# Luke-TS/3360-ray-tracer

Measured on AMD Instinct MI355X. Metric: Mrays/s (primary+secondary) at fixed spp; RMS pixel error vs CPU ref, higher is better.
Workload: dtype f64; 1 GPU; c3_bunny: bunny scene 1000x562, 200 spp, depth 20, fixed spp; scene_prims=69452, bvh_nodes=40541, mode=persistent, precision=fast, schedule=park, framebuffer=pinned host, frame_rows_covered=True, parallelism=tile-split x1 (interleaved 4-row stripes, no collectives)

## Files before the change

### 3360-ray-tracer_amd/csrc/rtx_device.h

```cpp
#pragma once

#include <hip/hip_runtime.h>
#include <stdint.h>

#include <type_traits>

#include "rtx.h"

#ifndef RTX_PARK_TU
#define RTX_PARK_TU 0
#endif

namespace rtxd {

constexpr bool kSincosSmall = !RTX_PARK_TU;
constexpr bool kTriBranchless = RTX_PARK_TU;
constexpr bool kEarlyTex = !RTX_PARK_TU;
constexpr bool kLeafStep = RTX_PARK_TU;

constexpr double kPi = 3.14159265358979323846;
constexpr double kInf = __builtin_inf();

struct V3 {
  double x, y, z;
// ... 333 lines not shown
  mat_out = R.mat;
  const PrimRec* P = &R;
  const int kind = KIND >= 0 ? KIND : P->kind;
  if (kTriBranchless && KIND >= 0 && kind == RTX_PRIM_TRIANGLE) {
    const V3 A{P->g[0], P->g[1], P->g[2]};
    const V3 e1 = tri_e1(P->g), e2 = tri_e2(P->g);
    const V3 pvec = cross(d, e2);
    const float det = (float)dot(e1, pvec);
    const float inv_det = 1.0f / det;
    const V3 tvec = o - A;
    const float u = (float)(dot(tvec, pvec) * (double)inv_det);
    const V3 qvec = cross(tvec, e1);
    const float v = (float)(dot(d, qvec) * (double)inv_det);
    const float t = (float)(dot(e2, qvec) * (double)inv_det);
    const bool ok = !(fabsf(det) < 1e-6f) & !(u < 0.0f || u > 1.0f) & !(v < 0.0f || (u + v) > 1.0f) &
                    !((double)t < tmin || (double)t > tmax);
    t_out = (double)t;
    return ok;
  }
  if (kind == RTX_PRIM_TRIANGLE) {
    V3 A{P->g[0], P->g[1], P->g[2]};
    V3 e1 = tri_e1(P->g), e2 = tri_e2(P->g);
    V3 pvec = cross(d, e2);
    float det = (float)dot(e1, pvec);
    if (fabsf(det) < 1e-6f) return false;
    float inv_det = 1.0f / det;
    V3 tvec = o - A;
    float u = (float)(dot(tvec, pvec) * (double)inv_det);
    if (u < 0.0f || u > 1.0f) return false;
    V3 qvec = cross(tvec, e1);
    float v = (float)(dot(d, qvec) * (double)inv_det);
    if (v < 0.0f || (u + v) > 1.0f) return false;
    float t = (float)(dot(e2, qvec) * (double)inv_det);
    if ((double)t < tmin || (double)t > tmax) return false;
    t_out = (double)t;
    return true;
  }
  if (kind == RTX_PRIM_SPHERE) {
    V3 c{P->g[0], P->g[1], P->g[2]};
    double radius = fmax(0.0, P->g[3]);
    V3 oc = c - o;
    double a = len2(d);
    double h = dot(d, oc);
    double cc = len2(oc) - radius * radius;
    double disc = h * h - a * cc;
    if (disc < 0) return false;
    double sq = sqrt(disc);
    double root = (h - sq) / a;
    if (!(tmin < root && root < tmax)) {
      root = (h + sq) / a;
      if (!(tmin < root && root < tmax)) return false;
    }
    t_out = root;
    return true;
  }
  int ax, a0, a1;
  if (kind == RTX_PRIM_XY_RECT) ax = 2, a0 = 0, a1 = 1;
  else if (kind == RTX_PRIM_XZ_RECT) ax = 1, a0 = 0, a1 = 2;
  else ax = 0, a0 = 1, a1 = 2;
  double t = (P->g[4] - comp(o, ax)) / comp(d, ax);
  if (!(tmin < t && t < tmax)) return false;
  double x = comp(o, a0) + t * comp(d, a0);
  double y = comp(o, a1) + t * comp(d, a1);
  if (x < P->g[0] || x > P->g[1] || y < P->g[2] || y > P->g[3]) return false;
  t_out = t;
  return true;
}

__device__ __forceinline__ bool prim_t(const rtx_prim* __restrict__ P, bool tris, V3 o, V3 d, double tmin,
                                       double tmax, double& t_out) {
  int32_t m;
  return prim_t(P, tris, o, d, tmin, tmax, t_out, m);
}

template <bool UV = true>
__device__ __forceinline__ void finish_hit(const DScene& S, int64_t best, V3 o, V3 d, double tmin, Hit& h) {
  h.u = 0.0, h.v = 0.0;
  hit_prim<UV>(S.prims + best, o, d, tmin, kInf, h);
  h.lazy_uv = (!UV && S.prims[best].kind == RTX_PRIM_SPHERE) ? best : -1;
}

template <bool UV = true>
__device__ __forceinline__ void finish_hit_at(const DScene& S, int64_t best, double t, V3 o, V3 d, Hit& h) {
  const rtx_prim* __restrict__ P = S.prims + best;
  const int kind = P->kind;
  h.u = 0.0, h.v = 0.0;
  h.mat = P->material;
  h.t = t;
  h.lazy_uv = -1;
  if (kind == RTX_PRIM_SPHERE) {
    const V3 c{P->g[0], P->g[1], P->g[2]};
    const double radius = fmax(0.0, P->g[3]);
    h.p = o + h.t * d;
    const V3 outward = (h.p - c) / radius;
    set_face_normal(h, d, outward);
    if (UV) sphere_uv(outward, h.u, h.v);
    else h.lazy_uv = best;
  } else if (kind == RTX_PRIM_TRIANGLE) {
    h.p = o + h.t * d;
    if (S.tri_n) {
      const double2 n01 = *(const double2*)(S.tri_n + 4 * best), n2 = *(const double2*)(S.tri_n + 4 * best + 2);
      set_face_normal(h, d, V3{n01.x, n01.y, n2.x});
    } else {
      const V3 e1 = tri_e1(P->g), e2 = tri_e2(P->g);
      set_face_normal(h, d, normalize(cross(e1, e2)));
    }
  } else {
    int a0, a1;
    V3 n;
    if (kind == RTX_PRIM_XY_RECT) a0 = 0, a1 = 1, n = v3(0, 0, 1);
    else if (kind == RTX_PRIM_XZ_RECT) a0 = 0, a1 = 2, n = v3(0, 1, 0);
    else a0 = 1, a1 = 2, n = v3(1, 0, 0);
    if (UV) {
      const double x = comp(o, a0) + t * comp(d, a0);
      const double y = comp(o, a1) + t * comp(d, a1);
      h.u = (x - P->g[0]) / (P->g[1] - P->g[0]);
      h.v = (y - P->g[2]) / (P->g[3] - P->g[2]);
    } else {
      h.lazy_uv = best;
    }
    set_face_normal(h, d, n);
    h.p = o + h.t * d;
  }
}

__device__ __forceinline__ bool box_hit(const double* lo, const double* hi, V3 o, V3 inv_unused, V3 d,
                                        double tmin, double tmax) {
#pragma unroll
  for (int a = 0; a < 3; a++) {
    const double adinv = 1.0 / comp(d, a);
    double t0 = (lo[a] - comp(o, a)) * adinv;
    double t1 = (hi[a] - comp(o, a)) * adinv;
    if (t0 < t1) {
      if (t0 > tmin) tmin = t0;
      if (t1 < tmax) tmax = t1;
    } else {
      if (t1 > tmin) tmin = t1;
      if (t0 < tmax) tmax = t0;
    }
    if (tmax <= tmin) return false;
  }
  return true;
}

struct Counters {
  uint32_t nodes, prims;
  uint32_t wnodes, wprims;
  uint32_t tris, sphs;
  uint32_t witers, widle;
  uint32_t wlive;
};
struct CountersClk : Counters {
  uint64_t t_top, t_seg, t_walk, t_leaf;
  uint64_t cyc_refill, cyc_walk, cyc_shade, cyc_leaf;
  uint32_t wshade, lshade;
};
__device__ __forceinline__ void count_prim(Counters& c, const rtx_prim* P) {
  c.prims++;
  const int k = P->kind;
  c.tris += k == RTX_PRIM_TRIANGLE ? 1u : 0u;
  c.sphs += k == RTX_PRIM_SPHERE ? 1u : 0u;
}
__device__ __forceinline__ bool first_active_lane() {
  const unsigned long long m = __ballot(1);
  return (int)__lane_id() == __ffsll((long long)m) - 1;
}

template <int STACK, bool COUNT>
__device__ __forceinline__ int64_t trace_parity(const DScene& S, V3 o, V3 d, double tmin, double tmax,
                                                uint32_t* stk, int stride, Counters& cnt, double& t_best) {
  int64_t best = -1;
  double closest = tmax, t;
  if (!S.use_bvh) {
    for (int64_t i = 0; i < S.n_prims; i++) {
      if (COUNT) count_prim(cnt, S.prims + i);
      if (prim_t(S.prims + i, S.has_tris, o, d, tmin, closest, t)) closest = t, best = i;
    }
    t_best = closest;
    return best;
  }
  int sp = 0;
  stk[0] = 0u;
  sp = 1;
  while (sp > 0) {
    const uint32_t ni = stk[(--sp) * stride];
    const rtx_bvh_node* __restrict__ nd = S.nodes + ni;
    double lo[3] = {nd->lo[0], nd->lo[1], nd->lo[2]};
    double hi[3] = {nd->hi[0], nd->hi[1], nd->hi[2]};
    const uint32_t a = nd->left_first, b = nd->right_count, leaf = nd->is_leaf;
    if (COUNT) cnt.nodes++;
    if (!box_hit(lo, hi, o, o, d, tmin, closest)) continue;
    if (leaf) {
      for (uint32_t i = 0; i < b; i++) {
        if (COUNT) count_prim(cnt, S.prims + a + i);
        if (prim_t(S.prims + a + i, S.has_tris, o, d, tmin, closest, t)) closest = t, best = (int64_t)a + i;
      }
    } else {
      if (sp + 2 > STACK) __builtin_trap();
      stk[(sp++) * stride] = b;
      stk[(sp++) * stride] = a;
    }
  }
  t_best = closest;
  return best;
}

__device__ __forceinline__ float f32_round_up(double x) {
  float f = (float)x;
  if ((double)f < x) f = __int_as_float(__float_as_int(f) + (f >= 0.0f ? 1 : -1));
  return f;
}

__device__ __forceinline__ void pin(double& x) { asm volatile("" : "+v"(x)); }
__device__ __forceinline__ void pin(V3& v) {
  pin(v.x);
  pin(v.y);
  pin(v.z);
}

__device__ __forceinline__ void fray4_axis_signed(double o, double d, int axis, float& inv, float& nl, float& nh,
                                                  uint32_t& off) {
  inv = __builtin_amdgcn_rcpf((float)d);
  const float n0 = -((float)o * inv);
  off = 32u * axis;
  if (!(fabsf(n0) < __builtin_inff())) {
    inv = 0.0f, nl = -__builtin_inff(), nh = __builtin_inff();
    return;
  }
  const float delta = fabsf(n0) * 0x1p-20f;
  nl = n0 - delta, nh = n0 + delta;
  if (inv < 0.0f) off += 16u;
}
__device__ __forceinline__ float f4c(const float4& v, int c) { return c == 0 ? v.x : (c == 1 ? v.y : (c == 2 ? v.z : v.w)); }

__device__ __forceinline__ void cswap4(float& ta, int32_t& ca, float& tb, int32_t& cb) {
  const bool s = tb < ta;
  const float t = s ? tb : ta;
  tb = s ? ta : tb;
  ta = t;
  const int32_t c = s ? cb : ca;
  cb = s ? ca : cb;
  ca = c;
}

struct FRay4L {
  float iex, iey, iez, nex, ney, nez;
  float ixx, ixy, ixz, nxx, nxy, nxz;
  uint32_t ox, oy, oz;
};
struct FRay4 {
  float ix, iy, iz, nlx, nhx, nly, nhy, nlz, nhz;
  uint32_t ox, oy, oz;
};
__device__ __forceinline__ FRay4L make_fray4l(V3 o, V3 d) {
  FRay4 b;
  fray4_axis_signed(o.x, d.x, 0, b.ix, b.nlx, b.nhx, b.ox);
  fray4_axis_signed(o.y, d.y, 1, b.iy, b.nly, b.nhy, b.oy);
  fray4_axis_signed(o.z, d.z, 2, b.iz, b.nlz, b.nhz, b.oz);
  constexpr float lo = 0.99999f, hi = 1.00001f;
  FRay4L r;
  r.iex = b.ix * lo, r.iey = b.iy * lo, r.iez = b.iz * lo;
  r.nex = b.nlx * lo, r.ney = b.nly * lo, r.nez = b.nlz * lo;
  r.ixx = b.ix * hi, r.ixy = b.iy * hi, r.ixz = b.iz * hi;
  r.nxx = b.nhx * hi, r.nxy = b.nhy * hi, r.nxz = b.nhz * hi;
  r.ox = b.ox, r.oy = b.oy, r.oz = b.oz;
  return r;
}

struct TravState {
  uint32_t node;
  int32_t sp;
  double closest;
  int32_t best;
  int32_t mat;
  float tmax_f;
};
__device__ __forceinline__ void trav_init(TravState& ts, double tmax) {
  ts.node = 0, ts.sp = 0, ts.closest = tmax, ts.best = -1, ts.mat = -1;
  ts.tmax_f = f32_round_up(tmax);
}

constexpr int32_t kGlobalSpheres = 4;
__device__ __forceinline__ bool sphere_root(double a, double h, double sq, double tmin, double tmax, double& root) {
  const double n1 = h - sq;
  const bool near_first = !(a > 0.0 && a < kInf && tmin >= 0.0) || n1 > 0.0;
  root = (near_first ? n1 : h + sq) / a;
  bool ok = tmin < root && root < tmax;
  if (!ok && near_first) {
    root = (h + sq) / a;
    ok = tmin < root && root < tmax;
  }
  return ok;
}
template <bool COUNT, bool SPHERES = true>
__device__ __forceinline__ void trav_globals(const DScene& S, V3 o, V3 d, double tmin, Counters& cnt, TravState& ts) {
  if (SPHERES && (S.n_global & kGlobalSpheres)) {
    typedef uint32_t u4 __attribute__((ext_vector_type(4)));
    typedef double d2 __attribute__((ext_vector_type(2)));
    typedef const __attribute__((address_space(4))) u4 cu4;
    typedef const __attribute__((address_space(4))) d2 cd2;
    for (int i = 0; i < (S.n_global & 3); i++) {
      const uintptr_t P = (uintptr_t)(S.prims + (uint32_t)S.global[i]);
      const u4 w0 = *(cu4*)P;
      const d2 w1 = *((cd2*)P + 1), w2 = *((cd2*)P + 2);
      if (COUNT) {
        cnt.prims++, cnt.sphs++;
// ... 291 lines not shown
}

__device__ __forceinline__ V3 tex_value(const DScene& S, int32_t t, const Hit& rec) {
  double u = rec.u, v = rec.v;
  const V3 p = rec.p;
  for (int guard = 0; guard < 16; guard++) {
    const rtx_texture T = S.texs[t];
    if (T.kind == RTX_TEX_SOLID) return v3(T.color[0], T.color[1], T.color[2]);
    if (T.kind == RTX_TEX_CHECKER) {
      int xi = (int)floor(T.inv_scale * p.x);
      int yi = (int)floor(T.inv_scale * p.y);
      int zi = (int)floor(T.inv_scale * p.z);
      t = ((xi + yi + zi) % 2 == 0) ? T.even : T.odd;
      continue;
    }
    if (T.image < 0) return v3(0, 1, 1);
    const DImage im = S.images[T.image];
    if (im.h <= 0) return v3(0, 1, 1);
    if (rec.lazy_uv >= 0) {
      const double2 uv = lazy_uv(S.prims + rec.lazy_uv, p);
      u = uv.x, v = uv.y;
    }
    u = u < 0 ? 0 : (u > 1 ? 1 : u);
    v = 1.0 - (v < 0 ? 0 : (v > 1 ? 1 : v));
    int i = (int)(u * im.w);
    int j = (int)(v * im.h);
    i = i < 0 ? 0 : (i < im.w ? i : im.w - 1);
    j = j < 0 ? 0 : (j < im.h ? j : im.h - 1);
    const uint8_t* px = im.texels + ((size_t)j * im.w + i) * 3;
    double s = 1.0 / 255.0;
    return v3(s * px[0], s * px[1], s * px[2]);
  }
  return v3(0, 1, 1);
}

__device__ __forceinline__ V3 mat_tex(const DScene& S, const rtx_material& m, const Hit& rec) {
  if (m.texture < 0) return v3(m.albedo[0], m.albedo[1], m.albedo[2]);
  return tex_value(S, m.texture, rec);
}

__device__ __forceinline__ double pow5(double x) {
  const double p2 = x * x, e2 = fma(x, x, -p2);
  const double p4 = p2 * p2, e4 = fma(p2, p2, -p4) + 2.0 * (p2 * e2);
  const double p5 = p4 * x, e5 = fma(p4, x, -p5) + e4 * x;
  return p5 + e5;
}

__device__ __forceinline__ double reflectance(double c, double ri) {
  double r0 = (1.0 - ri) / (1.0 + ri);
  r0 = r0 * r0;
  return r0 + (1.0 - r0) * pow5(1.0 - c);
}

__device__ __forceinline__ bool mat_scatter(const DScene& S, const rtx_material& m, V3 rin_d, const Hit& rec,
                                            V3& att, V3& sd, Rng& g) {
  if (m.kind == RTX_MAT_LAMBERTIAN) {
    V3 dir = rec.normal + random_unit_vector(g);
    if (near_zero(dir)) dir = rec.normal;
    sd = dir;
    att = mat_tex(S, m, rec);
    return true;
  }
  if (m.kind == RTX_MAT_METAL) {
    V3 r = reflect(rin_d, rec.normal);
    r = r + m.fuzz * random_unit_vector(g);
    sd = r;
    att = v3(m.albedo[0], m.albedo[1], m.albedo[2]);
    return dot(sd, rec.normal) > 0;
  }
  if (m.kind == RTX_MAT_DIELECTRIC) {
    att = v3(1.0, 1.0, 1.0);
    double eta = rec.front_face ? (1.0 / m.ref_idx) : m.ref_idx;
    V3 ud = normalize(rin_d);
    double ct = fmin(dot(-ud, rec.normal), 1.0);
    double stt = sqrt(1.0 - ct * ct);
    bool cannot = eta * stt > 1.0;
    if (cannot || reflectance(ct, eta) > g.next()) sd = reflect(ud, rec.normal);
    else sd = refract(ud, rec.normal, eta);
    return true;
  }
  return false;
}

__device__ __forceinline__ V3 mat_emitted(const DScene& S, const rtx_material& m, const Hit& rec) {
  if (m.kind == RTX_MAT_DIFFUSE_LIGHT) return mat_tex(S, m, rec);
  return v3(0, 0, 0);
}
template <bool NOTEX>
__device__ __forceinline__ V3 mat_tex_t(const DScene& S, const rtx_material& m, const Hit& rec) {
  if (NOTEX) return v3(m.albedo[0], m.albedo[1], m.albedo[2]);
  return mat_tex(S, m, rec);
}
template <bool NOTEX>
__device__ __forceinline__ V3 mat_emitted_t(const DScene& S, const rtx_material& m, const Hit& rec) {
  if (m.kind == RTX_MAT_DIFFUSE_LIGHT) return mat_tex_t<NOTEX>(S, m, rec);
  return v3(0, 0, 0);
}

__device__ __forceinline__ V3 sky(V3 d) {
  V3 ud = normalize(d);
  double t = 0.5 * (ud.y + 1.0);
  return (1.0 - t) * v3(1.0, 1.0, 1.0) + t * v3(0.5, 0.7, 1.0);
}

template <bool NODOF = false>
__device__ __forceinline__ void get_ray(const rtx_camera& c, int i, int j, Rng& g, V3& o, V3& d) {
  double oy = g.next() - 0.5;
  double ox = g.next() - 0.5;
  V3 p00{c.pixel00[0], c.pixel00[1], c.pixel00[2]};
  V3 du{c.pixel_delta_u[0], c.pixel_delta_u[1], c.pixel_delta_u[2]};
  V3 dv{c.pixel_delta_v[0], c.pixel_delta_v[1], c.pixel_delta_v[2]};
  V3 ps = p00 + ((i + ox) * du) + ((j + oy) * dv);
  V3 center{c.center[0], c.center[1], c.center[2]};
  if (NODOF || c.defocus_angle <= 0) {
    o = center;
  } else {
    V3 p = random_in_unit_disk(g);
    V3 ddu{c.defocus_disk_u[0], c.defocus_disk_u[1], c.defocus_disk_u[2]};
    V3 ddv{c.defocus_disk_v[0], c.defocus_disk_v[1], c.defocus_disk_v[2]};
    o = center + (p.x * ddu) + (p.y * ddv);
  }
  d = ps - o;
}

struct Path {
  V3 o, d, thr;
  int32_t depth;
};

__device__ __forceinline__ V3 normalize_l(V3 v, double& l) {
  l = sqrt(len2(v));
  if (l == 0.0) return {0, 0, 0};
  return v / l;
}

enum : int32_t {
  kShadeEmit = 0,
  kShadeDead = 1,
  kShadeDiffuse = 2,
  kShadeSpecular = 3
};
struct ShadeOut {
  V3 f;
  float ct, pdf;
  int32_t what;
  int32_t fsrc;
};
template <class T>
__device__ __forceinline__ const T* opaque(const T* p) {
  asm volatile("" : "+v"(p));
  return p;
}

template <bool LAMB = false, bool NOTEX = false, bool SET_ORIGIN = true, bool DEFER_F = false>
__device__ __forceinline__ void shade_core(const DScene& S, int max_depth, Path& p, const Hit& rec, bool hit, Rng& g,
                                           const rtx_material& m, ShadeOut& so) {
  static_assert(!DEFER_F || NOTEX, "deferred BSDF values need texture-free shading");
  so.what = kShadeDead;
  so.fsrc = 0;
  double lnd;
  const V3 nd = normalize_l(p.d, lnd);
  if (!hit || p.depth >= max_depth) {
    const double t = 0.5 * (nd.y + 1.0);
    so.f = (1.0 - t) * v3(1.0, 1.0, 1.0) + t * v3(0.5, 0.7, 1.0);
    so.what = kShadeEmit;
    return;
  }
  if (!LAMB) {
    V3 em = mat_emitted_t<NOTEX>(S, m, rec);
    if (!near_zero(em)) {
      so.f = em;
      so.what = kShadeEmit;
      return;
    }
  }
  const int kind = LAMB ? (int)RTX_MAT_LAMBERTIAN : m.kind;
  const bool isL = kind == RTX_MAT_LAMBERTIAN, isM = kind == RTX_MAT_METAL, isG = kind == RTX_MAT_DIELECTRIC;
  if (!(isL || isM || isG)) return;
  const V3 n = rec.normal;
  V3 ftex = v3(0, 0, 0);
  if (kEarlyTex && !NOTEX && !DEFER_F && isL) ftex = mat_tex_t<NOTEX>(S, m, rec);
  double r1 = 0.0, r2 = 0.0;
  if (isL) r1 = g.next(), r2 = g.next();
  V3 ru = v3(0, 0, 0);
  if (isM) ru = random_unit_vector(g);
  double l1;
  V3 s1 = normalize_l(isL ? n : nd, l1);
  pin(s1);
  const V3 w = s1;
  const V3 win = (!isL && l1 == 0.0) ? v3(-0.0, -0.0, -0.0) : s1;
  double eta = 0.0, ci = 0.0, a2 = 0.0;
  if (isG) {
    eta = rec.front_face ? m.albedo[0] : m.ref_idx;
    ci = dot(win, n);
    ci = ci < -1.0 ? -1.0 : (ci > 1.0 ? 1.0 : ci);
    a2 = fmax(0.0, 1.0 - ci * ci);
  }
  double s2 = sqrt(isL ? r2 : a2);
  pin(s2);
  double x = 0.0, y = 0.0;
  if (isL) {
    const double phi = 2.0 * kPi * r1;
    double cph, sph;
    cos_sin<kSincosSmall || !LAMB>(phi, cph, sph);
    x = s2 * cph;
    y = s2 * sph;
  }
  bool g_reflect = false;
  V3 perp = v3(0, 0, 0);
  double a3 = 1.0;
  if (isG) {
    const double st = eta * s2;
    g_reflect = st >= 1.0;
    if (!g_reflect) {
      const double r0 = m.albedo[1];
      const double Fr = r0 + (1.0 - r0) * pow5(1.0 - fabs(ci));
      g_reflect = g.next() < Fr;
    }
    if (!g_reflect) {
      const double c = fmin(dot(-win, n), 1.0);
      perp = eta * (win + c * n);
      a3 = fabs(1.0 - len2(perp));
    }
  }
  double s3 = sqrt(isL ? 1.0 - r2 : a3);
  pin(s3);
  V3 in4;
  if (isL) {
    const V3 a = (fabs(w.x) > 0.9) ? v3(0, 1, 0) : v3(1, 0, 0);
    in4 = cross(w, a);
  } else {
    in4 = reflect(nd, n);
    in4 = in4 + m.fuzz * ru;
  }
  double l4;
  V3 s4 = normalize_l(in4, l4);
  pin(s4);
  V3 wi;
  if (isL) {
    const V3 v = s4;
    const V3 u = cross(v, w);
    wi = normalize(x * u + y * v + s3 * w);
    if (dot(wi, n) <= 0) return;
    const float cf = (float)dot(n, wi);
    const float pdf = (cf <= 0.0f) ? 0.0f : (float)((double)cf / kPi);
    if (DEFER_F) so.fsrc = 1;
    else so.f = ((kEarlyTex && !NOTEX) ? ftex : mat_tex_t<NOTEX>(S, m, rec)) / kPi;
    if (pdf < 1e-6f) return;
    so.ct = fmaxf(0.0f, (float)dot(wi, n));
    so.pdf = pdf;
    so.what = kShadeDiffuse;
  } else if (isM) {
    wi = s4;
    if (dot(wi, n) <= 0) return;
    if (DEFER_F) so.fsrc = 2;
    else so.f = v3(m.albedo[0], m.albedo[1], m.albedo[2]);
    so.what = kShadeSpecular;
  } else {
    if (g_reflect) {
      wi = reflect(win, n);
      so.f = v3(1.0, 1.0, 1.0);
    } else {
      const V3 par = (-s3) * n;
      wi = perp + par;
      const double k = eta * eta;
      so.f = v3(k, k, k);
    }
    so.what = kShadeSpecular;
  }
  if (SET_ORIGIN) p.o = rec.p;
  p.d = wi, p.depth = p.depth + 1;
}

__device__ __forceinline__ bool shade_finish(const ShadeOut& so, V3& thr, int32_t depth, Rng& g, V3& L,
                                             const rtx_material* m = nullptr) {
  L = v3(0, 0, 0);
  if (so.what == kShadeEmit) {
    L = L + thr * so.f;
    return false;
  }
  if (so.what == kShadeDead) return false;
  V3 f = so.f;
  if (so.fsrc) {
    const rtx_material* mp = opaque(m);
    f = v3(mp->albedo[0], mp->albedo[1], mp->albedo[2]);
    if (so.fsrc == 1) f = f / kPi;
  }
  V3 c = so.what == kShadeDiffuse ? ((double)so.ct * (thr * f)) / (double)so.pdf : thr * f;
  if (depth > 5) {
    double q = fmax(fmax(c.x, c.y), c.z);
    q = q < 0.1 ? 0.1 : (q > 0.95 ? 0.95 : q);
    if (g.next() > q) return false;
    c = c / q;
  }
  thr = c;
  return true;
}

template <bool LAMB = false, bool NOTEX = false>
__device__ __forceinline__ bool shade_merged(const DScene& S, int max_depth, Path& p, const Hit& rec, bool hit,
                                             Rng& g, V3& L, const rtx_material& m) {
  ShadeOut so;
  shade_core<LAMB, NOTEX>(S, max_depth, p, rec, hit, g, m, so);
  return shade_finish(so, p.thr, p.depth, g, L);
}

template <bool LAMB = false, bool NOTEX = false>
__device__ __forceinline__ bool shade(const DScene& S, int max_depth, Path& p, const Hit& rec, bool hit, Rng& g,
                                      V3& L, const rtx_material& m) {
  return shade_merged<LAMB, NOTEX>(S, max_depth, p, rec, hit, g, L, m);
}

__device__ __forceinline__ bool shade(const DScene& S, int max_depth, Path& p, const Hit& rec, bool hit, Rng& g,
                                      V3& L) {
  rtx_material m;
  if (hit) m = S.mats[rec.mat];
  return shade(S, max_depth, p, rec, hit, g, L, m);
}

}
```

### 3360-ray-tracer_amd/csrc/rtx_kernels.h

```cpp
#pragma once

#include "rtx_device.h"

namespace rtxd {

constexpr int kBlock = 256;

constexpr int kTraceWaves = 4;
constexpr int kSlotTargetLog2 = 29;
constexpr int kRefillMin = 24;
constexpr int kRefillMinPark = 12;
constexpr int kParkAt = 16;
constexpr int kChunkPlain = 256, kChunkPark = 512;
constexpr int kChunkSharedPlain = 256, kChunkSharedPark = 128;
static_assert(kChunkSharedPlain <= 511 && kChunkSharedPark <= 511, "ChunkLds keeps a chunk's size in 9 bits");

struct FastDiv {
  uint32_t m, sh;
  __host__ __device__ __forceinline__ uint32_t div(uint32_t n) const {
    const uint32_t t = (uint32_t)(((uint64_t)n * m) >> 32);
    return (t + ((n - t) >> (sh & 0xFFu))) >> (sh >> 8);
  }
};
inline FastDiv make_fastdiv(uint32_t d) {
  if (d <= 1) return FastDiv{0u, 0u};
  uint32_t l = 0;
  while (l < 32 && (1ull << l) < d) l++;
  const uint64_t m = ((((uint64_t)1 << 32) * (((uint64_t)1 << l) - d)) / d) + 1;
  return FastDiv{(uint32_t)m, 1u | ((l - 1) << 8)};
}

struct PixelMap {
  int32_t W, H;
  int32_t stripes;
  int32_t x0, y0, w, h;
  int32_t srows, sidx, scount;
  FastDiv frow, fsrows;
  template <bool FD = true>
  __host__ __device__ __forceinline__ void xy(uint32_t local, int& x, int& y) const {
    if (!stripes) {
      const uint32_t r = FD ? frow.div(local) : local / (uint32_t)w;
      x = x0 + (int)(local - r * (uint32_t)w);
      y = y0 + (int)r;
    } else {
      const uint32_t r = FD ? frow.div(local) : local / (uint32_t)W;
      x = (int)(local - r * (uint32_t)W);
      const uint32_t blk = FD ? fsrows.div(r) : r / (uint32_t)srows;
      y = ((int)blk * scount + sidx) * srows + (int)(r - blk * (uint32_t)srows);
    }
  }
};
inline void set_map_div(PixelMap& m) {
  const int row = m.stripes ? m.W : m.w;
  m.frow = make_fastdiv((uint32_t)(row > 1 ? row : 1));
  m.fsrows = make_fastdiv((uint32_t)(m.srows > 1 ? m.srows : 1));
}

struct PathQueue {
  double *ox, *oy, *oz, *dx, *dy, *dz, *tx, *ty, *tz;
  uint32_t* slot;
  uint32_t* meta;
  int32_t* hit;
};

struct RenderArgs {
  DScene S;
  rtx_camera cam;
  PixelMap map;
  uint64_t seed;
  int64_t npix;
  int32_t K;
  FastDiv fK;
  int32_t s0;
  int32_t max_depth;
  int32_t scatter_api;
  const uint8_t* conv;
  double* L;
  unsigned long long* counters;
  int32_t stack_slots;
};

__device__ __forceinline__ void store_radiance(const RenderArgs& A, uint32_t slot, V3 L) {
  double* Lp = A.L + 3 * (uint64_t)slot;
  __builtin_nontemporal_store(L.x, Lp), __builtin_nontemporal_store(L.y, Lp + 1), __builtin_nontemporal_store(L.z, Lp + 2);
}

__device__ __forceinline__ uint32_t lane_id() { return __lane_id(); }

__device__ __forceinline__ int64_t wave_compact(bool want, unsigned int* counter) {
  const unsigned long long mask = __ballot(want);
  if (mask == 0) return -1;
  const int leader = __ffsll((long long)mask) - 1;
  const int total = __popcll(mask);
  unsigned int base = 0;
  if ((int)lane_id() == leader) base = atomicAdd(counter, (unsigned int)total);
  base = __shfl(base, leader);
  const int rank = __popcll(mask & ((1ull << lane_id()) - 1ull));
  return want ? (int64_t)base + rank : -1;
}

constexpr size_t stack_lds_bytes(int STACK) { return (size_t)(STACK + 1) * kBlock * sizeof(uint32_t); }
struct PersistLds {
  uint32_t stack, thr, hitp, leafq, block, end;
};

struct PixelSoA {
  double *sum, *mean, *m2;
  int32_t* samples;
  uint8_t* conv;
};

constexpr bool spec_walk(int park, bool fast, bool scatter) { return park == 2 && fast && !scatter; }
constexpr int64_t kSpecMaxNodes = 65536;
struct ChunkLds {
  unsigned long long w[kBlock / 64];
};
constexpr uint32_t block_region_bytes(int kind) { return kind == 1 ? (uint32_t)sizeof(ChunkLds) : 0u; }
constexpr int block_region_kind(int map, bool scatter) { return map == 1 && !scatter ? 1 : 0; }
constexpr PersistLds persist_lds(int stack_slots, bool spec, int block_region = 0) {
  const uint32_t stack_bytes = (uint32_t)stack_slots * kBlock * (spec ? 2u : 4u);
  const uint32_t thr = (stack_bytes + 7u) & ~7u, hitp = thr + 3u * kBlock * 8u, leafq = hitp + 3u * kBlock * 8u;
  const uint32_t tl = leafq + (spec ? (uint32_t)kLeafQueue * kBlock * 4u : 0u);
  return PersistLds{0u, thr, hitp, leafq, tl, tl + block_region_bytes(block_region)};
}

template <int STACK, bool FAST, bool COUNT, int TK = -1>
__device__ __forceinline__ int64_t trace(const DScene& S, V3 o, V3 d, double tmin, double tmax, uint32_t* stk,
                                         Counters& c, double& t_best, int32_t& mat_best) {
  if (FAST) return trace_fast4_lean<STACK, COUNT, TK>(S, o, d, tmin, tmax, stk, kBlock, c, t_best, mat_best);
  const int64_t b = trace_parity<STACK, COUNT>(S, o, d, tmin, tmax, stk, kBlock, c, t_best);
  mat_best = b >= 0 ? S.prims[b].material : -1;
  return b;
}
template <int STACK, bool FAST, bool COUNT>
__device__ __forceinline__ int64_t trace(const DScene& S, V3 o, V3 d, double tmin, double tmax, uint32_t* stk,
                                         Counters& c, double& t_best) {
  int32_t m;
  return trace<STACK, FAST, COUNT>(S, o, d, tmin, tmax, stk, c, t_best, m);
}

__device__ __forceinline__ void flush_clock(const RenderArgs& A, const CountersClk& c) {
  if (c.cyc_refill) atomicAdd(&A.counters[18], c.cyc_refill);
  if (c.cyc_walk) atomicAdd(&A.counters[19], c.cyc_walk);
  if (c.cyc_shade) atomicAdd(&A.counters[20], c.cyc_shade);
  if (c.wshade) atomicAdd(&A.counters[21], (unsigned long long)c.wshade);
  if (c.lshade) atomicAdd(&A.counters[22], (unsigned long long)c.lshade);
  if (c.cyc_leaf) atomicAdd(&A.counters[23], c.cyc_leaf);
}
__device__ __forceinline__ void flush_counters(const RenderArgs& A, const Counters& c, uint32_t segs,
                                               uint32_t prims, bool count) {
  if (count) {
    atomicAdd(&A.counters[2], (unsigned long long)c.nodes);
    atomicAdd(&A.counters[3], (unsigned long long)c.prims);
    atomicAdd(&A.counters[4], (unsigned long long)c.wnodes);
    atomicAdd(&A.counters[5], (unsigned long long)c.wprims);
    atomicAdd(&A.counters[6], (unsigned long long)c.tris);
    atomicAdd(&A.counters[7], (unsigned long long)c.sphs);
    if (c.witers) atomicAdd(&A.counters[10], (unsigned long long)c.witers);
    if (c.widle) atomicAdd(&A.counters[11], (unsigned long long)c.widle);
    if (c.wlive) atomicAdd(&A.counters[12], (unsigned long long)c.wlive);
  }
  if (segs) atomicAdd(&A.counters[0], (unsigned long long)segs);
  if (prims) atomicAdd(&A.counters[1], (unsigned long long)prims);
}

template <int STACK, bool FAST>
__global__ __launch_bounds__(kBlock, kTraceWaves) void k_intersect(DScene S, const rtx_ray* __restrict__ rays,
                                                                       int64_t n, rtx_hit* __restrict__ hits,
                                                                       double tmin, double tmax) {
  extern __shared__ __attribute__((aligned(16))) uint32_t lds[];
  uint32_t* stk = lds + threadIdx.x;
  const int64_t i = (int64_t)blockIdx.x * kBlock + threadIdx.x;
  if (i >= n) return;
  const rtx_ray r = rays[i];
  V3 o{r.origin[0], r.origin[1], r.origin[2]}, d{r.direction[0], r.direction[1], r.direction[2]};
  Counters c{};
  double tb;
  const int64_t best = trace<STACK, FAST, false>(S, o, d, tmin, tmax, stk, c, tb);
  rtx_hit out;
  out.pad_ = 0;
  if (best >= 0) {
    Hit h;
    finish_hit_at(S, best, tb, o, d, h);
    out.hit = 1;
    out.front_face = h.front_face, out.material = h.mat, out.t = h.t;
    out.p[0] = h.p.x, out.p[1] = h.p.y, out.p[2] = h.p.z;
    out.normal[0] = h.normal.x, out.normal[1] = h.normal.y, out.normal[2] = h.normal.z;
    out.u = h.u, out.v = h.v;
  } else {
    out.hit = 0, out.front_face = 0, out.material = -1, out.t = 0;
    out.p[0] = out.p[1] = out.p[2] = 0;
    out.normal[0] = out.normal[1] = out.normal[2] = 0;
    out.u = out.v = 0;
  }
  hits[i] = out;
}


template <int STACK, bool FAST, bool COUNT>
__global__ __launch_bounds__(kBlock, kTraceWaves) void k_wf_extend(RenderArgs A, PathQueue q,
                                                                       const unsigned int* count) {
  extern __shared__ __attribute__((aligned(16))) uint32_t lds[];
  uint32_t* stk = lds + threadIdx.x;
  const int64_t n = *count;
  Counters c{};
  uint32_t segs = 0;
  for (int64_t i = (int64_t)blockIdx.x * kBlock + threadIdx.x; i < n; i += (int64_t)gridDim.x * kBlock) {
    const V3 o = v3(q.ox[i], q.oy[i], q.oz[i]);
    const V3 d = v3(q.dx[i], q.dy[i], q.dz[i]);
    double tb;
    q.hit[i] = (int32_t)trace<STACK, FAST, COUNT>(A.S, o, d, (double)0.001f, kInf, stk, c, tb);
    segs++;
  }
  flush_counters(A, c, segs, 0, COUNT);
}



template <int STACK, bool FAST, bool COUNT, bool SCATTER, int PARK, int TK = -1, bool LAMB = false,
          bool NOTEX = false, bool NODOF = false, int MAP = 0>
__global__ __launch_bounds__(kBlock, kTraceWaves) void k_persistent(RenderArgs A, unsigned long long* next_slot) {
  extern __shared__ __attribute__((aligned(16))) uint32_t lds[];
  constexpr bool kSpecLds = spec_walk(PARK, FAST, SCATTER);
  constexpr bool kShared = block_region_kind(MAP, SCATTER) == 1;
  static_assert((PARK > 0) == (RTX_PARK_TU != 0), "k_persistent: PARK kernels belong to rtx_park.hip");
  constexpr int kChunk = PARK ? kChunkPark : kChunkPlain;
  constexpr int kChunkShared = PARK ? kChunkSharedPark : kChunkSharedPlain;
  const PersistLds lay = persist_lds(A.stack_slots, kSpecLds, block_region_kind(MAP, SCATTER));
  char* const ldsb = (char*)lds;
  if (COUNT && threadIdx.x == 0) atomicMax(&A.counters[13], ~(unsigned long long)wall_clock64());
  unsigned long long* const cw = (unsigned long long*)(ldsb + lay.block);
  (void)cw;
  if (kShared) {
    if (threadIdx.x < kBlock / 64) cw[threadIdx.x] = 0ull;
    __syncthreads();
  }
  uint32_t* stk = (uint32_t*)(ldsb + lay.stack) + threadIdx.x;
  uint16_t* stk16 = (uint16_t*)(ldsb + lay.stack) + threadIdx.x;
  (void)stk16;
  double* thr_lds = (double*)(ldsb + lay.thr) + threadIdx.x;
  double* hitp_lds = (double*)(ldsb + lay.hitp) + threadIdx.x;
  uint32_t* leafq = (uint32_t*)(ldsb + lay.leafq) + threadIdx.x;
  (void)leafq;
  constexpr bool kHitpLds = (NOTEX || kEarlyTex) && !SCATTER;
  (void)hitp_lds;
  const uint64_t nslots = MAP == 1 ? (uint64_t)next_slot[8 * 16] : (uint64_t)A.npix * (uint64_t)A.K;
  const double tmin = SCATTER ? 0.001 : (double)0.001f;
  std::conditional_t<COUNT, CountersClk, Counters> c{};
  uint32_t segs = 0, prims = 0;
  uint32_t pseg = 0;
  uint16_t* const segbuf = !COUNT ? nullptr : (uint16_t*)next_slot[8 * 16 + 4];
  (void)pseg, (void)segbuf;
  uint64_t chunk_base = 0, chunk_left = 0;
  bool exhausted = false;
  bool dry = false;
  uint32_t region = blockIdx.x & 7;
  bool has = false;
  Path P;
  P.depth = 0;
  uint32_t slot = 0;
  uint32_t pix = 0, smp = 0;
  constexpr bool kPark = PARK > 0 && FAST && !SCATTER;
  const bool park_ok = kPark && A.S.use_bvh && !A.S.froot_leaf;
  bool parked = false;
  TravState trs;
  while (true) {
    if constexpr (COUNT) {
      const uint64_t now = __builtin_amdgcn_s_memtime();
      const unsigned long long tw = __ballot(c.t_walk != 0);
      if (c.t_seg && tw) {
        const uint64_t w = __shfl(c.t_walk, __ffsll((long long)tw) - 1);
        if (lane_id() == 0) c.cyc_refill += c.t_seg - c.t_top, c.cyc_walk += w - c.t_seg, c.cyc_shade += now - w;
      } else if (c.t_top && lane_id() == 0) {
        c.cyc_refill += now - c.t_top;
      }
      c.t_top = now, c.t_seg = 0, c.t_walk = 0;
    }
    const unsigned long long idle = __ballot(!has);
    bool fresh = false;
    constexpr int kRefill = kPark ? kRefillMinPark : kRefillMin;
    if (kShared) {
      if (idle != 0 && !exhausted && (__popcll(idle) >= kRefill || idle == ~0ull)) {
        const uint32_t nidle = (uint32_t)__popcll(idle);
        const uint32_t rank = (uint32_t)__popcll(idle & ((1ull << lane_id()) - 1ull));
        const int wv = (int)(threadIdx.x >> 6);
        uint32_t given = 0;
        auto take = [&](int j) {
          unsigned long long old = 0;
          if (lane_id() == 0) old = atomicAdd(&cw[j], (unsigned long long)(nidle - given));
          old = __shfl(old, 0);
          const uint32_t cs = (uint32_t)(old >> 32), csz = ((uint32_t)old >> 23) & 0x1FFu, cur = (uint32_t)old & 0x7FFFFFu;
          const uint32_t got = cur < csz ? min(nidle - given, csz - cur) : 0u;
          if (!has && rank >= given && rank < given + got) slot = cs + cur + (rank - given), fresh = true;
          given += got;
        };
        take(wv);
        if (given < nidle && !dry) {
          bool ok = false;
          for (int tries = 0; tries < 8 && !ok; tries++) {
            unsigned long long b = 0;
            if (lane_id() == 0) b = atomicAdd(next_slot + 16 * region, (unsigned long long)kChunkShared);
            b = __shfl(b, 0);
            const uint64_t rs = ((uint64_t)region * nslots) >> 3, re = ((uint64_t)(region + 1) * nslots) >> 3;
            if (rs + b < re) {
              ok = true;
              const uint32_t csz = (uint32_t)min<uint64_t>(kChunkShared, re - (rs + b));
              if (lane_id() == 0) atomicExch(&cw[wv], ((unsigned long long)(rs + b) << 32) | ((unsigned long long)csz << 23));
            } else {
              region = (region + 1) & 7;
            }
          }
          if (ok) take(wv);
          else dry = true;
        }
        for (int m = 1; m < kBlock / 64 && dry && given < nidle; m++) take((wv + m) & (kBlock / 64 - 1));
        if (dry && given == 0) {
          exhausted = true;
          if (COUNT && lane_id() == 0) {
            const unsigned long long t = (unsigned long long)wall_clock64();
            atomicMax(&A.counters[14], t);
            atomicMax(&A.counters[15], ~t);
          }
        }
      }
    } else if (idle != 0 && !exhausted && (__popcll(idle) >= kRefill || idle == ~0ull)) {
      const uint64_t nidle = (uint64_t)__popcll(idle);
      const uint64_t rank = (uint64_t)__popcll(idle & ((1ull << lane_id()) - 1ull));
      uint64_t cand = ~0ull;
      if (chunk_left >= nidle) {
        if (!has) cand = chunk_base + rank;
        chunk_base += nidle, chunk_left -= nidle;
      } else {
        uint64_t nb = ~0ull, ne = 0;
        for (int tries = 0; tries < 8 && nb == ~0ull; tries++) {
          unsigned long long b = 0;
          if (lane_id() == 0) b = atomicAdd(next_slot + 16 * region, (unsigned long long)kChunk);
          b = __shfl(b, 0);
          const uint64_t rs = ((uint64_t)region * nslots) >> 3, re = ((uint64_t)(region + 1) * nslots) >> 3;
          if (rs + b < re) nb = rs + b, ne = std::min<uint64_t>(rs + b + kChunk, re);
          else region = (region + 1) & 7;
        }
        if (!has) {
          if (rank < chunk_left) cand = chunk_base + rank;
          else if (nb != ~0ull && nb + (rank - chunk_left) < ne) cand = nb + (rank - chunk_left);
        }
        if (nb != ~0ull) {
          const uint64_t used = std::min<uint64_t>(nidle - chunk_left, ne - nb);
          chunk_base = nb + used, chunk_left = (ne - nb) - used;
        } else {
          chunk_left = 0, exhausted = true;
          if (COUNT && lane_id() == 0) {
            const unsigned long long t = (unsigned long long)wall_clock64();
            atomicMax(&A.counters[14], t);
            atomicMax(&A.counters[15], ~t);
          }
        }
      }
      if (cand < nslots) slot = (uint32_t)cand, fresh = true;
    }
    if (fresh) {
      constexpr bool kArgsAtRefill = !(LAMB && NOTEX);
      auto kseg = __builtin_amdgcn_kernarg_segment_ptr();
      if (kArgsAtRefill) asm volatile("" : "+s"(kseg));
      const RenderArgs& Ar = kArgsAtRefill ? *(const RenderArgs*)kseg : A;
      if (COUNT && kArgsAtRefill && (Ar.npix != A.npix || Ar.seed != A.seed || Ar.stack_slots != A.stack_slots))
        __builtin_trap();
      constexpr bool kFdMap1 = false;
      uint2 e = make_uint2(0u, 0u);
      if (MAP == 1) {
        const uint2* const sm = (const uint2*)next_slot[8 * 16 + 2];
        if (sm) {
          e = sm[slot];
        } else {
          const uint32_t q = kFdMap1 ? Ar.fK.div(slot) : slot / (uint32_t)Ar.K;
          e = make_uint2(q, (uint32_t)Ar.s0 + (slot - q * (uint32_t)Ar.K));
        }
      }
      const uint32_t p = MAP ? e.x : Ar.fK.div(slot);
      if (!(Ar.conv && Ar.conv[p])) {
        const int k = MAP ? 0 : (int)((uint32_t)slot - p * (uint32_t)Ar.K);
        int x, y;
        Ar.map.template xy<MAP == 0 || kFdMap1>(p, x, y);
        pix = (uint32_t)(y * Ar.map.W + x), smp = MAP ? e.y : (uint32_t)(Ar.s0 + k);
        Rng g = make_rng(A.seed, pix, smp, 0u);
        get_ray<NODOF>(Ar.cam, x, y, g, P.o, P.d);
        thr_lds[0] = 1.0, thr_lds[kBlock] = 1.0, thr_lds[2 * kBlock] = 1.0;
        P.depth = SCATTER ? Ar.max_depth : 0;
        has = true;
        prims++;
        if (COUNT) pseg = 0;
      }
    }
    if (COUNT && lane_id() == 0) c.witers++;
    if (!__any(has)) {
      if (COUNT && lane_id() == 0) c.widle++;
      if (exhausted) break;
      continue;
    }
    if (COUNT) {
      const uint32_t live = (uint32_t)__popcll(__ballot(has));
      if (lane_id() == 0) c.wlive += live;
    }
    if constexpr (COUNT) c.t_seg = __builtin_amdgcn_s_memtime();
    if (!has) continue;
    __builtin_amdgcn_s_setprio(1);
    V3 L;
    bool cont;
    if (SCATTER && P.depth <= 0) {
      L = v3(0, 0, 0);
      cont = false;
    } else {
      double tb;
      int32_t bmat;
      int64_t best;
      if (kPark && park_ok) {
        const int active = __popcll(__ballot(1));
        if (!parked) {
          trav_init(trs, kInf);
          constexpr bool kGlobalSph = !(PARK == 1 && TK >= 0 && LAMB && NOTEX && MAP == 0);
          trav_globals<COUNT, kGlobalSph>(A.S, P.o, P.d, tmin, c, trs);
        }
        const bool done =
            kSpecLds ? trace4_run_spec<STACK, COUNT, TK>(A.S, P.o, P.d, tmin, stk16, leafq, kBlock, c, trs,
                                                         active > kParkAt ? kParkAt : -1)
                     : trace4_run<STACK, COUNT, TK>(A.S, P.o, P.d, tmin, stk, kBlock, c, trs,
                                                    active > kParkAt ? kParkAt : -1);
        parked = !done;
        if constexpr (COUNT) c.t_walk = __builtin_amdgcn_s_memtime();
        if (parked) continue;
        best = trs.best, tb = trs.closest, bmat = trs.mat;
      } else if (kPark) {
        best = trace_flat(A.S, P.o, P.d, tmin, kInf, c, COUNT, tb, bmat);
      } else {
        best = trace<STACK, FAST, COUNT, TK>(A.S, P.o, P.d, tmin, kInf, stk, c, tb, bmat);
      }
      segs++;
      if constexpr (COUNT) {
        pseg++;
        if (!kPark || !park_ok) c.t_walk = __builtin_amdgcn_s_memtime();
        const unsigned long long sh = __ballot(1);
        if ((int)lane_id() == __ffsll((long long)sh) - 1) c.wshade++, c.lshade += (uint32_t)__popcll(sh);
      }
      __builtin_amdgcn_s_setprio(0);
      Hit h;
      rtx_material m;
      if (best >= 0) finish_hit_at<false>(A.S, best, tb, P.o, P.d, h);
      if (kHitpLds && best >= 0) hitp_lds[0] = h.p.x, hitp_lds[kBlock] = h.p.y, hitp_lds[2 * kBlock] = h.p.z;
      if (best >= 0) m = A.S.mats[h.mat];
      if (SCATTER) P.thr = v3(thr_lds[0], thr_lds[kBlock], thr_lds[2 * kBlock]);
      Rng g = make_rng(A.seed, pix, smp, SCATTER ? (uint32_t)(A.max_depth - P.depth) + 1u : (uint32_t)P.depth + 1u);
      if (SCATTER) {
        if (best < 0) {
          L = P.thr * sky(P.d);
          cont = false;
        } else {
          V3 att, sd;
          if (mat_scatter(A.S, m, P.d, h, att, sd, g)) {
            P.thr = P.thr * att;
            P.o = h.p, P.d = sd;
            P.depth--;
            cont = true;
          } else {
            L = P.thr * mat_emitted(A.S, m, h);
            cont = false;
          }
        }
        if (cont) thr_lds[0] = P.thr.x, thr_lds[kBlock] = P.thr.y, thr_lds[2 * kBlock] = P.thr.z;
      } else {
        ShadeOut so;
        const rtx_material& mr = *opaque(A.S.mats + (best >= 0 ? h.mat : 0));
        shade_core<LAMB, NOTEX, !kHitpLds>(A.S, A.max_depth, P, h, best >= 0, g, mr, so);
        V3 thr = v3(thr_lds[0], thr_lds[kBlock], thr_lds[2 * kBlock]);
        cont = shade_finish(so, thr, P.depth, g, L, best >= 0 ? A.S.mats + h.mat : A.S.mats);
        if (cont) thr_lds[0] = thr.x, thr_lds[kBlock] = thr.y, thr_lds[2 * kBlock] = thr.z;
        if (kHitpLds && cont) P.o = v3(hitp_lds[0], hitp_lds[kBlock], hitp_lds[2 * kBlock]);
      }
    }
    if (!cont) {
      store_radiance(A, slot, L);
      if (COUNT && segbuf) segbuf[slot] = (uint16_t)min(pseg, 65535u);
      has = false;
    }
  }
  flush_counters(A, c, segs, prims, COUNT);
  if constexpr (COUNT) flush_clock(A, c);
  if (COUNT && lane_id() == 0) {
    const unsigned long long t = (unsigned long long)wall_clock64();
    atomicMax(&A.counters[16], t);
    atomicMax(&A.counters[17], ~t);
  }
}

#define RTX_PARK_INSTANCES(X)                                                                                    \
  X(32, false, false, 0, 1) X(32, true, false, 0, 1) X(64, false, false, 0, 1)                                  \
  X(64, true, false, 0, 1) X(32, false, true, 0, 1) X(32, true, true, 0, 1)                                     \
  X(64, false, true, 0, 1) X(64, true, true, 0, 1) X(32, false, false, 1, 1)                                    \
  X(32, true, false, 1, 1) X(64, false, false, 1, 1) X(64, true, false, 1, 1)                                   \
  X(32, false, false, 0, 2) X(32, true, false, 0, 2) X(64, false, false, 0, 2)                                  \
  X(64, true, false, 0, 2) X(32, false, false, 1, 2) X(32, true, false, 1, 2)                                   \
  X(64, false, false, 1, 2) X(64, true, false, 1, 2)
#define RTX_PARK_TRI_INSTANCES(Y) Y(32, 0, 1) Y(64, 0, 1) Y(32, 1, 1) Y(64, 1, 1) Y(32, 0, 2) Y(64, 0, 2) Y(32, 1, 2) Y(64, 1, 2)


}
```

Baseline: 12510 Mrays/s.

## Defer hit shading in park mode until enough lanes are pending

In the persistent park kernel, lanes that finish traversal with a hit now record the hit in the traversal state and mark themselves pending instead of shading at once. The wave shades only when at least a threshold of lanes are pending (default 24), when the work supply is exhausted, or when the remaining lanes cannot trigger a refill. Misses and depth-limited paths are resolved inline with a cheap sky term. The aim is to cut divergence in the shading phase by running it on fuller waves. The cost is that lanes can sit idle while pending, plus extra ballots each loop iteration.

```diff
diff --git a/3360-ray-tracer_amd/csrc/rtx_device.h b/3360-ray-tracer_amd/csrc/rtx_device.h
--- a/3360-ray-tracer_amd/csrc/rtx_device.h
+++ b/3360-ray-tracer_amd/csrc/rtx_device.h
@@ -509,6 +509,7 @@
 };
 struct CountersClk : Counters {
   uint64_t t_top, t_seg, t_walk, t_leaf;
+  uint64_t t_sh;
   uint64_t cyc_refill, cyc_walk, cyc_shade, cyc_leaf;
   uint32_t wshade, lshade;
 };
@@ -1106,6 +1107,22 @@
   return p;
 }
 
+__device__ __forceinline__ void shade_sky_end(V3 nd, ShadeOut& so) {
+  const double t = 0.5 * (nd.y + 1.0);
+  so.f = (1.0 - t) * v3(1.0, 1.0, 1.0) + t * v3(0.5, 0.7, 1.0);
+  so.what = kShadeEmit;
+}
+__device__ __forceinline__ V3 shade_emit(const ShadeOut& so, V3 thr) {
+  V3 L = v3(0, 0, 0);
+  return L + thr * so.f;
+}
+__device__ __forceinline__ V3 shade_terminal(V3 d, V3 thr) {
+  double lnd;
+  ShadeOut so;
+  shade_sky_end(normalize_l(d, lnd), so);
+  return shade_emit(so, thr);
+}
+
 template <bool LAMB = false, bool NOTEX = false, bool SET_ORIGIN = true, bool DEFER_F = false>
 __device__ __forceinline__ void shade_core(const DScene& S, int max_depth, Path& p, const Hit& rec, bool hit, Rng& g,
                                            const rtx_material& m, ShadeOut& so) {
@@ -1115,9 +1132,7 @@
   double lnd;
   const V3 nd = normalize_l(p.d, lnd);
   if (!hit || p.depth >= max_depth) {
-    const double t = 0.5 * (nd.y + 1.0);
-    so.f = (1.0 - t) * v3(1.0, 1.0, 1.0) + t * v3(0.5, 0.7, 1.0);
-    so.what = kShadeEmit;
+    shade_sky_end(nd, so);
     return;
   }
   if (!LAMB) {
@@ -1230,7 +1245,7 @@
                                              const rtx_material* m = nullptr) {
   L = v3(0, 0, 0);
   if (so.what == kShadeEmit) {
-    L = L + thr * so.f;
+    L = shade_emit(so, thr);
     return false;
   }
   if (so.what == kShadeDead) return false;
diff --git a/3360-ray-tracer_amd/csrc/rtx_kernels.h b/3360-ray-tracer_amd/csrc/rtx_kernels.h
--- a/3360-ray-tracer_amd/csrc/rtx_kernels.h
+++ b/3360-ray-tracer_amd/csrc/rtx_kernels.h
@@ -11,6 +11,11 @@
 constexpr int kRefillMin = 24;
 constexpr int kRefillMinPark = 12;
 constexpr int kParkAt = 16;
+#ifndef RTX_SHADE_MIN
+#define RTX_SHADE_MIN 24
+#endif
+constexpr int kShadeMinPark = RTX_SHADE_MIN;
+static_assert(kShadeMinPark >= 1 && kShadeMinPark <= 64, "lanes of a wave");
 constexpr int kChunkPlain = 256, kChunkPark = 512;
 constexpr int kChunkSharedPlain = 256, kChunkSharedPark = 128;
 static_assert(kChunkSharedPlain <= 511 && kChunkSharedPark <= 511, "ChunkLds keeps a chunk's size in 9 bits");
@@ -264,8 +269,62 @@
   const bool park_ok = kPark && A.S.use_bvh && !A.S.froot_leaf;
   bool parked = false;
   TravState trs;
+  constexpr int kRefill = kPark ? kRefillMinPark : kRefillMin;
+  constexpr int kShade = kPark && MAP == 0 ? kShadeMinPark : 1;
+  constexpr bool kBatch = kShade > 1;
+  constexpr uint32_t kPendNode = 0xFFFFFFFFu;
+  if (kBatch) trs.node = 0;
+  auto end_path = [&](V3 L) {
+    store_radiance(A, slot, L);
+    if (COUNT && segbuf) segbuf[slot] = (uint16_t)min(pseg, 65535u);
+    has = false;
+  };
+  auto shade_segment = [&](int64_t best, double tb, V3& L) -> bool {
+    bool cont;
+    Hit h;
+    rtx_material m;
+    if (best >= 0) finish_hit_at<false>(A.S, best, tb, P.o, P.d, h);
+    if (kHitpLds && best >= 0) hitp_lds[0] = h.p.x, hitp_lds[kBlock] = h.p.y, hitp_lds[2 * kBlock] = h.p.z;
+    if (best >= 0) m = A.S.mats[h.mat];
+    if (SCATTER) P.thr = v3(thr_lds[0], thr_lds[kBlock], thr_lds[2 * kBlock]);
+    Rng g = make_rng(A.seed, pix, smp, SCATTER ? (uint32_t)(A.max_depth - P.depth) + 1u : (uint32_t)P.depth + 1u);
+    if (SCATTER) {
+      if (best < 0) {
+        L = P.thr * sky(P.d);
+        cont = false;
+      } else {
+        V3 att, sd;
+        if (mat_scatter(A.S, m, P.d, h, att, sd, g)) {
+          P.thr = P.thr * att;
+          P.o = h.p, P.d = sd;
+          P.depth--;
+          cont = true;
+        } else {
+          L = P.thr * mat_emitted(A.S, m, h);
+          cont = false;
+        }
+      }
+      if (cont) thr_lds[0] = P.thr.x, thr_lds[kBlock] = P.thr.y, thr_lds[2 * kBlock] = P.thr.z;
+    } else {
+      ShadeOut so;
+      const rtx_material& mr = *opaque(A.S.mats + (best >= 0 ? h.mat : 0));
+      shade_core<LAMB, NOTEX, !kHitpLds>(A.S, A.max_depth, P, h, best >= 0, g, mr, so);
+      V3 thr = v3(thr_lds[0], thr_lds[kBlock], thr_lds[2 * kBlock]);
+      cont = shade_finish(so, thr, P.depth, g, L, best >= 0 ? A.S.mats + h.mat : A.S.mats);
+      if (cont) thr_lds[0] = thr.x, thr_lds[kBlock] = thr.y, thr_lds[2 * kBlock] = thr.z;
+      if (kHitpLds && cont) P.o = v3(hitp_lds[0], hitp_lds[kBlock], hitp_lds[2 * kBlock]);
+    }
+    return cont;
+  };
   while (true) {
-    if constexpr (COUNT) {
+    if constexpr (COUNT && kBatch) {
+      const uint64_t now = __builtin_amdgcn_s_memtime();
+      if (lane_id() == 0) {
+        if (c.t_seg) c.cyc_refill += c.t_seg - c.t_sh, c.cyc_walk += now - c.t_seg;
+        else if (c.t_top) c.cyc_refill += now - c.t_sh;
+      }
+      c.t_top = now, c.t_sh = now, c.t_seg = 0;
+    } else if constexpr (COUNT) {
       const uint64_t now = __builtin_amdgcn_s_memtime();
       const unsigned long long tw = __ballot(c.t_walk != 0);
       if (c.t_seg && tw) {
@@ -276,9 +335,32 @@
       }
       c.t_top = now, c.t_seg = 0, c.t_walk = 0;
     }
+    if constexpr (kBatch) {
+      const bool pend = has && trs.node == kPendNode;
+      const unsigned long long pm = __ballot(pend);
+      if (pm != 0) {
+        const int np = __popcll(pm), ni = __popcll(__ballot(!has));
+        if (np >= kShade || exhausted || (np + ni == 64 && ni < kRefill)) {
+          __builtin_amdgcn_s_setprio(0);
+          if (pend) {
+            if constexpr (COUNT) {
+              if ((int)lane_id() == __ffsll((long long)pm) - 1) c.wshade++, c.lshade += (uint32_t)np;
+            }
+            V3 L;
+            const bool cont = shade_segment(trs.best, trs.closest, L);
+            trs.node = 0;
+            if (!cont) end_path(L);
+          }
+          if constexpr (COUNT) {
+            const uint64_t t = __builtin_amdgcn_s_memtime();
+            if (lane_id() == 0) c.cyc_shade += t - c.t_top;
+            c.t_sh = t;
+          }
+        }
+      }
+    }
     const unsigned long long idle = __ballot(!has);
     bool fresh = false;
-    constexpr int kRefill = kPark ? kRefillMinPark : kRefillMin;
     if (kShared) {
       if (idle != 0 && !exhausted && (__popcll(idle) >= kRefill || idle == ~0ull)) {
         const uint32_t nidle = (uint32_t)__popcll(idle);
@@ -402,7 +484,7 @@
       if (lane_id() == 0) c.wlive += live;
     }
     if constexpr (COUNT) c.t_seg = __builtin_amdgcn_s_memtime();
-    if (!has) continue;
+    if (!has || (kBatch && trs.node == kPendNode)) continue;
     __builtin_amdgcn_s_setprio(1);
     V3 L;
     bool cont;
@@ -438,49 +520,25 @@
       if constexpr (COUNT) {
         pseg++;
         if (!kPark || !park_ok) c.t_walk = __builtin_amdgcn_s_memtime();
-        const unsigned long long sh = __ballot(1);
-        if ((int)lane_id() == __ffsll((long long)sh) - 1) c.wshade++, c.lshade += (uint32_t)__popcll(sh);
+        if constexpr (!kBatch) {
+          const unsigned long long sh = __ballot(1);
+          if ((int)lane_id() == __ffsll((long long)sh) - 1) c.wshade++, c.lshade += (uint32_t)__popcll(sh);
+        }
       }
       __builtin_amdgcn_s_setprio(0);
-      Hit h;
-      rtx_material m;
-      if (best >= 0) finish_hit_at<false>(A.S, best, tb, P.o, P.d, h);
-      if (kHitpLds && best >= 0) hitp_lds[0] = h.p.x, hitp_lds[kBlock] = h.p.y, hitp_lds[2 * kBlock] = h.p.z;
-      if (best >= 0) m = A.S.mats[h.mat];
-      if (SCATTER) P.thr = v3(thr_lds[0], thr_lds[kBlock], thr_lds[2 * kBlock]);
-      Rng g = make_rng(A.seed, pix, smp, SCATTER ? (uint32_t)(A.max_depth - P.depth) + 1u : (uint32_t)P.depth + 1u);
-      if (SCATTER) {
-        if (best < 0) {
-          L = P.thr * sky(P.d);
+      if constexpr (kBatch) {
+        if (best < 0 || P.depth >= A.max_depth) {
+          L = shade_terminal(P.d, v3(thr_lds[0], thr_lds[kBlock], thr_lds[2 * kBlock]));
           cont = false;
         } else {
-          V3 att, sd;
-          if (mat_scatter(A.S, m, P.d, h, att, sd, g)) {
-            P.thr = P.thr * att;
-            P.o = h.p, P.d = sd;
-            P.depth--;
-            cont = true;
-          } else {
-            L = P.thr * mat_emitted(A.S, m, h);
-            cont = false;
-          }
-        }
-        if (cont) thr_lds[0] = P.thr.x, thr_lds[kBlock] = P.thr.y, thr_lds[2 * kBlock] = P.thr.z;
+          trs.best = (int32_t)best, trs.closest = tb, trs.node = kPendNode;
+          cont = true;
+        }
       } else {
-        ShadeOut so;
-        const rtx_material& mr = *opaque(A.S.mats + (best >= 0 ? h.mat : 0));
-        shade_core<LAMB, NOTEX, !kHitpLds>(A.S, A.max_depth, P, h, best >= 0, g, mr, so);
-        V3 thr = v3(thr_lds[0], thr_lds[kBlock], thr_lds[2 * kBlock]);
-        cont = shade_finish(so, thr, P.depth, g, L, best >= 0 ? A.S.mats + h.mat : A.S.mats);
-        if (cont) thr_lds[0] = thr.x, thr_lds[kBlock] = thr.y, thr_lds[2 * kBlock] = thr.z;
-        if (kHitpLds && cont) P.o = v3(hitp_lds[0], hitp_lds[kBlock], hitp_lds[2 * kBlock]);
-      }
-    }
-    if (!cont) {
-      store_radiance(A, slot, L);
-      if (COUNT && segbuf) segbuf[slot] = (uint16_t)min(pseg, 65535u);
-      has = false;
-    }
+        cont = shade_segment(best, tb, L);
+      }
+    }
+    if (!cont) end_path(L);
   }
   flush_counters(A, c, segs, prims, COUNT);
   if constexpr (COUNT) flush_clock(A, c);
```

After: 13120 Mrays/s (median of 6 runs). 4.9% higher.
